# OpenVVC/OpenVVC

Hardware: AMD Instinct MI355X
Metric: decoded frames/sec, full rcn back-end decode step (H2D of the recorded picture + MC incl. BDOF/DMVR/affine-PROF/GPM/CIIP + LMCS + inverse transform + ordered intra pass + deblocking + SAO + ALF/CC-ALF + D2H of refined MVs + wait + per-picture digest + publication to the device DPB), 4K 10-bit RA rec (higher is better)
Workload: dtype u16 samples / int16 coefficients / int32 accumulate

## Files before the change

openvvc_amd/csrc/kernels_alf.hip:

```cpp
#include "ovvc_common.hip.h"

#ifndef OV_WPE_ALF
#define OV_WPE_ALF 0
#endif
#if OV_WPE_ALF > 0
#define OV_OCC_ALF __attribute__((amdgpu_waves_per_eu(OV_WPE_ALF)))
#else
#define OV_OCC_ALF
#endif

namespace {

#define TL 32
#define LH 3
#define LW (TL + 2 * LH)
#define LPAD 4
#define LWS 40
#define CH 2
#define CW (TL + 2 * CH)

struct AlfRect { int x0, y0, x1, y1; };
__device__ __forceinline__ AlfRect alf_clamp_rect(int border, int x0, int y0, int s, int w, int h)
{
    AlfRect r = { 0, 0, w - 1, h - 1 };
    if (border & OVHIP_BORDER_LEFT) r.x0 = x0;
    if (border & OVHIP_BORDER_UPPER) r.y0 = y0;
    if (border & OVHIP_BORDER_RIGHT) r.x1 = min(r.x1, x0 + s - 1);
    if (border & OVHIP_BORDER_BOTTOM) r.y1 = min(r.y1, y0 + s - 1);
    return r;
}

__device__ __forceinline__ int alf_clipd(int clip, int ref, int a, int b)
{
    return ov_clip3(a - ref, -clip, clip) + ov_clip3(b - ref, -clip, clip);
}

typedef short alf_s2 __attribute__((ext_vector_type(2)));
#define A6I(c) (((c) + 4) >> 1)
#define A6H(c) (((c) + 4) & 1)
#define A2I(c) ((c) >> 1)
#define A2H(c) ((c) & 1)
#define ALF_PK(da, ha, db, hb) __builtin_amdgcn_perm((db), (da), (uint32_t)((2 * (ha)) | ((2 * (ha) + 1) << 8) | ((4 + 2 * (hb)) << 16) | ((5 + 2 * (hb)) << 24)))
#define ALF_PK66(A, ca, B, cb) ALF_PK((A)[A6I(ca)], A6H(ca), (B)[A6I(cb)], A6H(cb))
#define ALF_PK22(A, ca, B, cb) ALF_PK((A)[A2I(ca)], A2H(ca), (B)[A2I(cb)], A2H(cb))
__device__ __forceinline__ uint32_t alf_dup(int v) { return __builtin_amdgcn_perm((uint32_t)v, (uint32_t)v, 0x01000100u); }
__device__ __forceinline__ int alf_tap(uint32_t pair, uint32_t cur2, uint32_t c2, uint32_t nc2, uint32_t f2, int sum)
{
    alf_s2 d = __builtin_bit_cast(alf_s2, pair) - __builtin_bit_cast(alf_s2, cur2);
    d = __builtin_elementwise_min(__builtin_elementwise_max(d, __builtin_bit_cast(alf_s2, nc2)), __builtin_bit_cast(alf_s2, c2));
    return __builtin_amdgcn_sdot2(d, __builtin_bit_cast(alf_s2, f2), sum, false);
}
__device__ __forceinline__ int alf_tap_lin(uint32_t pair, uint32_t f2, int sum)
{
    return __builtin_amdgcn_sdot2(__builtin_bit_cast(alf_s2, pair), __builtin_bit_cast(alf_s2, f2), sum, false);
}

__device__ __forceinline__ void filter_idx(uint32_t sum_h, uint32_t sum_v, uint32_t sum_d, uint32_t sum_b, bool is_vb,
                                           int &cls, int &tr)
{
    const uint32_t scale = is_vb ? 96u : 64u;
    const int act = min((int)(((sum_h + sum_v) * scale) >> (OV_BD + 4)), 15);
    int c = act == 0 ? 0 : act == 1 ? 1 : act <= 6 ? 2 : act <= 14 ? 3 : 4;
    uint32_t max_hv, min_hv, max_db, min_db, max_dir, min_dir;
    int dir_hv, dir_db, main_dir, sec_dir;
    if (sum_v > sum_h) { max_hv = sum_v; min_hv = sum_h; dir_hv = 1; } else { max_hv = sum_h; min_hv = sum_v; dir_hv = 3; }
    if (sum_d > sum_b) { max_db = sum_d; min_db = sum_b; dir_db = 0; } else { max_db = sum_b; min_db = sum_d; dir_db = 2; }
    if (max_db * min_hv > max_hv * min_db) { max_dir = max_db; min_dir = min_db; main_dir = dir_db; sec_dir = dir_hv; }
    else { max_dir = max_hv; min_dir = min_hv; main_dir = dir_hv; sec_dir = dir_db; }
    if (max_dir * 2 > 9 * min_dir) c += (((main_dir & 1) << 1) + 2) * 5;
    else if (max_dir > 2 * min_dir) c += (((main_dir & 1) << 1) + 1) * 5;
    cls = c;
    const int k = (main_dir << 1) + (sec_dir >> 1);
    tr = (0xDE84 >> (2 * k)) & 3;
}

__device__ __forceinline__ void alf_luma_tile(const ovhip_pic &dst, const ovhip_pic &src, const ovhip_alf_pic &alf, int nb_ctu_w,
                                              int tile0, uint16_t *s_t, uint8_t *s_cls, uint4 *s_sum, int row0, int row1)
{

    const int W = src.w, H = src.h;
    const int tid = threadIdx.x;
    const int ctu = 1 << alf.log2_ctu_s;
    const int ntx = (W + TL - 1) / TL, ntiles = ntx * ((H + TL - 1) / TL);
    for (int tile = tile0; tile < ntiles; tile = ntiles) {
    const int tx0 = (tile % ntx) * TL, ty0 = (tile / ntx) * TL;
    const ovhip_alf_ctu c = alf.ctus[(ty0 >> alf.log2_ctu_s) * nb_ctu_w + (tx0 >> alf.log2_ctu_s)];
    const bool on = c.flags & 4;

    const int b = tid >> 2, r = tid & 3;
    const int bx = (b & 7) * 4, by = (b >> 3) * 4;
    const int ox = tx0 + bx, oy = ty0 + by + r;

    if (!on) {
        if (oy < H && oy >= row0 && oy < row1) {
#pragma unroll
            for (int i = 0; i < 4; ++i) if (ox + i < W) dst.y[oy * dst.stride_y + ox + i] = src.y[oy * src.stride_y + ox + i];
        }
        continue;
    }

    const AlfRect rc = alf_clamp_rect(c.border, tx0 & ~(ctu - 1), ty0 & ~(ctu - 1), ctu, W, H);
    if (tx0 >= rc.x0 + LPAD && tx0 + TL + LPAD <= rc.x1 + 1 && ty0 >= rc.y0 + LH && ty0 + TL + LH <= rc.y1 + 1 && !(src.stride_y & 7)) {
        if (tid < LW * 5) {
            const int yy = tid / 5, q = tid - yy * 5;
            *reinterpret_cast<uint4 *>(s_t + yy * LWS + 8 * q) =
                *reinterpret_cast<const uint4 *>(src.y + (ty0 + yy - LH) * src.stride_y + tx0 - LPAD + 8 * q);
        }
    } else {
        for (int i = tid; i < LW * LWS; i += 256) {
            const int yy = i / LWS, xx = i - yy * LWS;
            const int sy = ov_clip3(ty0 + yy - LH, rc.y0, rc.y1), sx = ov_clip3(tx0 + xx - LPAD, rc.x0, rc.x1);
            s_t[i] = src.y[sy * src.stride_y + sx];
        }
    }
    __syncthreads();

    const int ctu_y0 = ty0 & ~(ctu - 1);
    const bool truncated = ctu_y0 + ctu > H;
    const int vbl = truncated ? H : ctu - 4;
    const int last_local = (ctu_y0 + (truncated ? H - ctu_y0 : ctu) - 1) & (ctu - 1);
    const bool req_vb = (last_local < vbl && last_local >= vbl - 4) || (last_local >= vbl && last_local <= vbl + 3);
    const int vb = ctu_y0 + vbl;

#define T(x, y) ((int)s_t[((y) + LH) * LWS + (x) + LPAD])
    {
        const int cb = tid >> 2, k = tid & 3;
        const int cbx = (cb & 7) * 4, cby = (cb >> 3) * 4;
        const int rr = cby - 2 + 2 * k;
        int above = rr - 1, below = rr + 2;
        if (ty0 + rr + 2 == vb) below = rr + 1;
        if (ty0 + rr == vb)     above = rr;
        uint32_t sv = 0, sh = 0, sd = 0, sb = 0;
        {
            uint32_t ra[6], r0[6], r1[6], rb[6];
            const uint16_t *base = s_t + LH * LWS + cbx;
            auto row3 = [&](int y, uint32_t d6[6]) {
                const uint2 *q2 = reinterpret_cast<const uint2 *>(base + y * LWS);
                const uint2 a = q2[0], b_ = q2[1], c_ = q2[2];
                d6[0] = a.x; d6[1] = a.y; d6[2] = b_.x; d6[3] = b_.y; d6[4] = c_.x; d6[5] = c_.y;
            };
            row3(above, ra); row3(rr, r0); row3(rr + 1, r1); row3(below, rb);
            typedef unsigned short alf_u2 __attribute__((ext_vector_type(2)));
#pragma unroll
            for (int q = 0; q < 4; ++q) {
                const int c0 = 2 * q - 2, c1 = c0 + 1;
                const alf_u2 ctr = __builtin_bit_cast(alf_u2, ALF_PK66(r0, c0, r1, c1));
                const uint32_t y2 = __builtin_bit_cast(uint32_t, ctr + ctr);
#define LAP(acc, A, ca, B, cb, C, cc_, D, cd)                                                                      \
                acc = __builtin_amdgcn_sad_u16(y2, __builtin_bit_cast(uint32_t, __builtin_bit_cast(alf_u2, ALF_PK66(A, ca, B, cb)) + \
                                                                               __builtin_bit_cast(alf_u2, ALF_PK66(C, cc_, D, cd))), acc)
                LAP(sv, ra, c0, r0, c1, r1, c0, rb, c1);
                LAP(sh, r0, c0 + 1, r1, c1 + 1, r0, c0 - 1, r1, c1 - 1);
                LAP(sd, ra, c0 - 1, r0, c1 - 1, r1, c0 + 1, rb, c1 + 1);
                LAP(sb, r1, c0 - 1, rb, c1 - 1, ra, c0 + 1, r0, c1 + 1);
#undef LAP
            }
        }
        const int py = ty0 + cby;
        bool use = true, is_vb = false;
        if (py == vb - 4) { is_vb = true; use = k < 3; }
        if (py == vb)     { is_vb = true; use = k > 0; }
        if (!use) sv = sh = sd = sb = 0;
        (void)is_vb;
        s_sum[tid] = make_uint4(sv, sh, sd, sb);
    }
    __syncthreads();
    if (tid < 64) {
        const uint4 p0 = s_sum[4 * tid], p1 = s_sum[4 * tid + 1], p2 = s_sum[4 * tid + 2], p3 = s_sum[4 * tid + 3];
        const int py = ty0 + (tid >> 3) * 4;
        int cls, tr;
        filter_idx(p0.y + p1.y + p2.y + p3.y, p0.x + p1.x + p2.x + p3.x, p0.z + p1.z + p2.z + p3.z, p0.w + p1.w + p2.w + p3.w,
                   py == vb - 4 || py == vb, cls, tr);
        s_cls[tid] = (uint8_t)(cls | (tr << 5));
    }
    __syncthreads();

    if (oy >= H || oy < row0 || oy >= row1) continue;
    const int ct = s_cls[b];
    const int cls = ct & 31, tr = ct >> 5;
    const int16_t *f = alf.luma_coeff + c.luma_set * OVHIP_ALF_LUMA_SET_SIZE + tr * 25 * 13 + cls * 13;
    const int16_t *cl = alf.luma_clip + c.luma_set * OVHIP_ALF_LUMA_SET_SIZE + tr * 25 * 13 + cls * 13;
    typedef uint32_t alf_u32a2 __attribute__((aligned(2)));
    uint32_t fw[6], cw6[6];
#pragma unroll
    for (int j = 0; j < 6; ++j) { fw[j] = *reinterpret_cast<const alf_u32a2 *>(f + 2 * j); cw6[j] = *reinterpret_cast<const alf_u32a2 *>(cl + 2 * j); }

    int d = 3;
    bool near = false;
    if (req_vb) {
        if (oy < vb && oy >= vb - 4) d = vb - 1 - oy;
        else if (oy >= vb && oy <= vb + 3) d = oy - vb;
        near = (oy == vb - 1) || (oy == vb);
    }
    const int o1 = min(d, 1), o2 = min(d, 2), o3 = min(d, 3);
    const int ly = by + r;
    uint32_t r0[6], p1[6], m1[6], p2[6], m2[6], p3[2], m3[2];
    {
        const uint16_t *base = s_t + LH * LWS + bx;
        auto row3 = [&](int y, uint32_t d6[6]) {
            const uint2 *q = reinterpret_cast<const uint2 *>(base + y * LWS);
            const uint2 a = q[0], b_ = q[1], c_ = q[2];
            d6[0] = a.x; d6[1] = a.y; d6[2] = b_.x; d6[3] = b_.y; d6[4] = c_.x; d6[5] = c_.y;
        };
        auto row1 = [&](int y, uint32_t d2[2]) {
            const uint2 a = reinterpret_cast<const uint2 *>(base + y * LWS)[1];
            d2[0] = a.x; d2[1] = a.y;
        };
        row3(ly, r0); row3(ly + o1, p1); row3(ly - o1, m1); row3(ly + o2, p2); row3(ly - o2, m2);
        row1(ly + o3, p3); row1(ly - o3, m3);
    }
#define S6(d6, c) ((((c) + 4) & 1) ? (int)((d6)[((c) + 4) >> 1] >> 16) : (int)((d6)[((c) + 4) >> 1] & 0xffff))
#define S2(d2, c) (((c) & 1) ? (int)((d2)[(c) >> 1] >> 16) : (int)((d2)[(c) >> 1] & 0xffff))
    alf_s2 cm2 = __builtin_bit_cast(alf_s2, cw6[0]);
    int fsum = 0;
#pragma unroll
    for (int j = 1; j < 6; ++j) cm2 = __builtin_elementwise_min(cm2, __builtin_bit_cast(alf_s2, cw6[j]));
#pragma unroll
    for (int j = 0; j < 6; ++j) fsum = __builtin_amdgcn_sdot2(__builtin_bit_cast(alf_s2, fw[j]), (alf_s2)(1), fsum, false);
    const int cmin = min((int)cm2.x, (int)cm2.y);
    const bool linear = __all(cmin > OV_PIX_MAX);
    uint32_t f2[12], c2[12], nc2[12];
#pragma unroll
    for (int j = 0; j < 6; ++j) {
        f2[2 * j] = __builtin_amdgcn_perm(fw[j], fw[j], 0x01000100u); f2[2 * j + 1] = __builtin_amdgcn_perm(fw[j], fw[j], 0x03020302u);
    }
    if (!linear) {
#pragma unroll
        for (int j = 0; j < 6; ++j) {
            c2[2 * j] = __builtin_amdgcn_perm(cw6[j], cw6[j], 0x01000100u); c2[2 * j + 1] = __builtin_amdgcn_perm(cw6[j], cw6[j], 0x03020302u);
        }
#pragma unroll
        for (int i = 0; i < 12; ++i) nc2[i] = __builtin_bit_cast(uint32_t, (alf_s2)(0) - __builtin_bit_cast(alf_s2, c2[i]));
    }
    int outv[4];
#pragma unroll
    for (int i = 0; i < 4; ++i) {
        const int cur = S6(r0, i);
        const uint32_t n[12] = {
            ALF_PK22(p3, i, m3, i),
            ALF_PK66(p2, i + 1, m2, i - 1), ALF_PK66(p2, i, m2, i), ALF_PK66(p2, i - 1, m2, i + 1),
            ALF_PK66(p1, i + 2, m1, i - 2), ALF_PK66(p1, i + 1, m1, i - 1), ALF_PK66(p1, i, m1, i),
            ALF_PK66(p1, i - 1, m1, i + 1), ALF_PK66(p1, i - 2, m1, i + 2),
            ALF_PK66(r0, i + 3, r0, i - 3), ALF_PK66(r0, i + 2, r0, i - 2), ALF_PK66(r0, i + 1, r0, i - 1) };
        int sum;
        if (linear) {
            sum = -2 * cur * fsum;
#pragma unroll
            for (int k = 0; k < 12; ++k) sum = alf_tap_lin(n[k], f2[k], sum);
        } else {
            const uint32_t cur2 = ALF_PK66(r0, i, r0, i);
            sum = 0;
#pragma unroll
            for (int k = 0; k < 12; ++k) sum = alf_tap(n[k], cur2, c2[k], nc2[k], f2[k], sum);
        }
        sum = near ? (sum + 512) >> 10 : (sum + 64) >> 7;
        outv[i] = ov_clip_bd(sum + cur);
    }
#undef S6
#undef S2
    {
        uint16_t *o = dst.y + oy * dst.stride_y + ox;
        if (ox + 3 < W && !(dst.stride_y & 3)) {
            uint2 v; v.x = (uint32_t)outv[0] | ((uint32_t)outv[1] << 16); v.y = (uint32_t)outv[2] | ((uint32_t)outv[3] << 16);
            *reinterpret_cast<uint2 *>(o) = v;
        } else {
#pragma unroll
            for (int i = 0; i < 4; ++i) if (ox + i < W) o[i] = (uint16_t)outv[i];
        }
    }
    }
#undef T
}

__device__ __forceinline__ void alf_chroma_tile(const ovhip_pic &dst, const ovhip_pic &src, const ovhip_alf_pic &alf, int nb_ctu_w,
                                                int tile0, int comp, uint16_t *s_t, int row0, int row1)
{
    const int W = src.w, H = src.h, Wc = W >> 1, Hc = H >> 1;
    const int tid = threadIdx.x;
    const int ctu = 1 << alf.log2_ctu_s, ctuc = ctu >> 1;
    const int ntx = (Wc + TL - 1) / TL, ntiles = ntx * ((Hc + TL - 1) / TL);
    for (int tile = tile0; tile < ntiles; tile = ntiles) {
    const int tx0 = (tile % ntx) * TL, ty0 = (tile / ntx) * TL;
    const ovhip_alf_ctu c = alf.ctus[((ty0 * 2) >> alf.log2_ctu_s) * nb_ctu_w + ((tx0 * 2) >> alf.log2_ctu_s)];
    const bool on = c.flags & (comp == 1 ? 2 : 1);
    const int cc_idx = comp == 1 ? c.cc_cb_idx : c.cc_cr_idx;
    const uint16_t *sp = comp == 1 ? src.cb : src.cr;
    uint16_t *dp = comp == 1 ? dst.cb : dst.cr;

    const AlfRect rcc = alf_clamp_rect(c.border, tx0 & ~(ctuc - 1), ty0 & ~(ctuc - 1), ctuc, Wc, Hc);
    if (on) {
        if (tx0 >= rcc.x0 + LPAD && tx0 + TL + LPAD <= rcc.x1 + 1 && ty0 >= rcc.y0 + CH && ty0 + TL + CH <= rcc.y1 + 1 && !(src.stride_c & 7)) {
            if (tid < CW * 5) {
                const int yy = tid / 5, q = tid - yy * 5;
                *reinterpret_cast<uint4 *>(s_t + yy * LWS + 8 * q) =
                    *reinterpret_cast<const uint4 *>(sp + (ty0 + yy - CH) * src.stride_c + tx0 - LPAD + 8 * q);
            }
        } else {
            for (int i = tid; i < CW * LWS; i += 256) {
                const int yy = i / LWS, xx = i - yy * LWS;
                const int sy = ov_clip3(ty0 + yy - CH, rcc.y0, rcc.y1), sx = ov_clip3(tx0 + xx - LPAD, rcc.x0, rcc.x1);
                s_t[i] = sp[sy * src.stride_c + sx];
            }
        }
        __syncthreads();
    }

    const int ctu_y0 = (ty0 * 2) & ~(ctu - 1);
    const bool truncated = ctu_y0 + ctu > H;
    int fc[6], cl[6];
    if (on) {
        const int alt = comp == 1 ? c.cb_alt : c.cr_alt;
#pragma unroll
        for (int i = 0; i < 6; ++i) { fc[i] = alf.chroma_coeff[alt * 7 + i]; cl[i] = alf.chroma_clip[alt * 7 + i]; }
    }
    int cf[7];
    if (cc_idx) {
#pragma unroll
        for (int i = 0; i < 7; ++i) cf[i] = alf.cc_coeff[((comp - 1) * 4 + (cc_idx - 1)) * 8 + i];
    }

    const int ly = tid >> 3, lx0 = (tid & 7) * 4;
    const int oy = ty0 + ly;
    if (oy >= Hc || oy < (row0 >> 1) || oy >= (row1 >> 1)) continue;
    int o1 = 1, o2 = 2;
    bool near = false;
    if (on) {
        const int vb = truncated ? H / 2 : (ctu - 4) / 2;
        const int yl = oy & (ctuc - 1);
        int d = 2;
        if (yl < vb && yl >= vb - 2) d = vb - 1 - yl;
        else if (yl >= vb && yl <= vb + 1) d = yl - vb;
        near = (yl == vb - 1) || (yl == vb);
        o1 = min(d, 1); o2 = min(d, 2);
    }
    int r1 = 1, r2 = -1, r3 = 2;
    if (cc_idx) {
        const int vbpos = truncated ? H / 2 : ctu - 4;
        const int pos = (oy << 1) & (ctu - 1);
        if (pos == vbpos - 2 || pos == vbpos + 1) r3 = r1;
        else if (pos == vbpos - 1 || pos == vbpos) r1 = r2 = r3 = 0;
    }
    const bool cc_inside = tx0 > rcc.x0 && ty0 > rcc.y0 && tx0 + TL <= rcc.x1 && ty0 + TL <= rcc.y1;
    const AlfRect rcl = { 2 * rcc.x0, 2 * rcc.y0, min(2 * rcc.x1 + 1, W - 1), min(2 * rcc.y1 + 1, H - 1) };
    uint32_t r0[6], p1[6], m1[6], p2[2], m2[2];
    int cmin = 0x7fff, fsum = 0;
    if (on) {
        const uint16_t *base = s_t + CH * LWS + lx0;
        auto row3 = [&](int y, uint32_t d6[6]) {
            const uint2 *q = reinterpret_cast<const uint2 *>(base + y * LWS);
            const uint2 a = q[0], b_ = q[1], c_ = q[2];
            d6[0] = a.x; d6[1] = a.y; d6[2] = b_.x; d6[3] = b_.y; d6[4] = c_.x; d6[5] = c_.y;
        };
        auto row1 = [&](int y, uint32_t d2[2]) {
            const uint2 a = reinterpret_cast<const uint2 *>(base + y * LWS)[1];
            d2[0] = a.x; d2[1] = a.y;
        };
        row3(ly, r0); row3(ly + o1, p1); row3(ly - o1, m1); row1(ly + o2, p2); row1(ly - o2, m2);
#pragma unroll
        for (int i = 0; i < 6; ++i) { cmin = min(cmin, cl[i]); fsum += fc[i]; }
    }
    const bool linear = on && cmin > OV_PIX_MAX;
    uint32_t f2[6], c2[6], nc2[6];
#pragma unroll
    for (int i = 0; i < 6; ++i) {
        f2[i] = alf_dup(fc[i]);
        c2[i] = alf_dup(cl[i]);
        nc2[i] = __builtin_bit_cast(uint32_t, (alf_s2)(0) - __builtin_bit_cast(alf_s2, c2[i]));
    }
#define S6(d6, c) ((((c) + 4) & 1) ? (int)((d6)[((c) + 4) >> 1] >> 16) : (int)((d6)[((c) + 4) >> 1] & 0xffff))
#define S2(d2, c) (((c) & 1) ? (int)((d2)[(c) >> 1] >> 16) : (int)((d2)[(c) >> 1] & 0xffff))
    int outv[4];
#pragma unroll
    for (int i = 0; i < 4; ++i) {
        const int ox = min(tx0 + lx0 + i, Wc - 1);
        int out;
        if (on) {
            const int cur = S6(r0, i);
            int sum;
            const uint32_t n[6] = { ALF_PK22(p2, i, m2, i),
                                    ALF_PK66(p1, i + 1, m1, i - 1), ALF_PK66(p1, i, m1, i), ALF_PK66(p1, i - 1, m1, i + 1),
                                    ALF_PK66(r0, i + 2, r0, i - 2), ALF_PK66(r0, i + 1, r0, i - 1) };
            if (linear) {
                sum = -2 * cur * fsum;
#pragma unroll
                for (int k = 0; k < 6; ++k) sum = alf_tap_lin(n[k], f2[k], sum);
            } else {
                const uint32_t cur2 = ALF_PK66(r0, i, r0, i);
                sum = 0;
#pragma unroll
                for (int k = 0; k < 6; ++k) sum = alf_tap(n[k], cur2, c2[k], nc2[k], f2[k], sum);
            }
            sum = near ? (sum + 512) >> 10 : (sum + 64) >> 7;
            out = ov_clip_bd(sum + cur);
        } else {
            out = sp[oy * src.stride_c + ox];
        }
        if (cc_idx) {
            const int Lx = ox << 1, Ly = oy << 1;
            int cy, sum = 0;
            if (cc_inside) {
                const uint16_t *lp = src.y + Ly * src.stride_y + Lx;
                cy = lp[0];
                sum += cf[0] * ((int)lp[r2 * src.stride_y] - cy);
                sum += cf[1] * ((int)lp[-1] - cy);
                sum += cf[2] * ((int)lp[1] - cy);
                sum += cf[3] * ((int)lp[r1 * src.stride_y - 1] - cy);
                sum += cf[4] * ((int)lp[r1 * src.stride_y] - cy);
                sum += cf[5] * ((int)lp[r1 * src.stride_y + 1] - cy);
                sum += cf[6] * ((int)lp[r3 * src.stride_y] - cy);
            } else {
#define LU(dx, dy) ((int)src.y[ov_clip3(Ly + (dy), rcl.y0, rcl.y1) * src.stride_y + ov_clip3(Lx + (dx), rcl.x0, rcl.x1)])
                cy = LU(0, 0);
                sum += cf[0] * (LU(0, r2) - cy);
                sum += cf[1] * (LU(-1, 0) - cy);
                sum += cf[2] * (LU(1, 0) - cy);
                sum += cf[3] * (LU(-1, r1) - cy);
                sum += cf[4] * (LU(0, r1) - cy);
                sum += cf[5] * (LU(1, r1) - cy);
                sum += cf[6] * (LU(0, r3) - cy);
#undef LU
            }
            sum = (sum + 64) >> 7;
            sum = ov_clip_bd(sum + (1 << OV_BD >> 1));
            out = ov_clip_bd(sum + out - (1 << OV_BD >> 1));
        }
        outv[i] = out;
    }
#undef S6
#undef S2
    uint16_t *o = dp + oy * dst.stride_c + tx0 + lx0;
    if (tx0 + lx0 + 3 < Wc && !(dst.stride_c & 3)) {
        uint2 v; v.x = (uint32_t)outv[0] | ((uint32_t)outv[1] << 16); v.y = (uint32_t)outv[2] | ((uint32_t)outv[3] << 16);
        *reinterpret_cast<uint2 *>(o) = v;
    } else {
#pragma unroll
        for (int i = 0; i < 4; ++i) if (tx0 + lx0 + i < Wc) o[i] = (uint16_t)outv[i];
    }
    }
}

__global__ __launch_bounds__(256) OV_OCC_ALF void k_alf(ovhip_pic dst, ovhip_pic src, ovhip_alf_pic alf, int nb_ctu_w, int nl, int nc, int t0_l, int t0_c, int row0, int row1)
{
    __shared__ __attribute__((aligned(16))) uint16_t s_t[(LW > CW ? LW : CW) * LWS];
    __shared__ uint8_t s_cls[64];
    __shared__ __attribute__((aligned(16))) uint4 s_sum[256];
    const int b = blockIdx.x;
    if (b < nl) alf_luma_tile(dst, src, alf, nb_ctu_w, t0_l + (int)ov_xcd_slot_at(b, 0, nl), s_t, s_cls, s_sum, row0, row1);
    else {
        const int comp = 1 + (b - nl) / nc;
        alf_chroma_tile(dst, src, alf, nb_ctu_w, t0_c + (int)ov_xcd_slot_at(b, nl + (comp - 1) * nc, nc), comp, s_t, row0, row1);
    }
}

}

extern "C" int ovhip_alf_launch_rows(ovhip_ctx *ctx, const ovhip_pic *dst, const ovhip_pic *src, const ovhip_alf_pic *alf, int32_t row0, int32_t row1)
{
    if (!ctx || !dst || !src || !alf) return OVHIP_EINVAL;
    OV_DEVICE(ctx);
    if (dst->w != src->w || dst->h != src->h || dst->y == src->y || alf->log2_ctu_s < 6 || alf->log2_ctu_s > 7 ||
        !alf->ctus || !alf->luma_coeff || !alf->luma_clip || !alf->chroma_coeff || !alf->chroma_clip || !alf->cc_coeff)
        return ov_fail(ctx, OVHIP_EINVAL, "ovhip_alf_launch: bad pictures / parameter tables", hipSuccess);
    if (row0 < 0 || row1 > src->h || row0 > row1 || (row0 & 7) || ((row1 & 7) && row1 != src->h))
        return ov_fail(ctx, OVHIP_EINVAL, "ovhip_alf_launch_rows: row window", hipSuccess);
    if (row0 == row1) return OVHIP_OK;
    const int nb_ctu_w = (src->w + (1 << alf->log2_ctu_s) - 1) >> alf->log2_ctu_s;
    const int ntx_l = (src->w + TL - 1) / TL, ntx_c = (src->w / 2 + TL - 1) / TL;
    const int ty0_l = row0 / TL, ty1_l = (row1 + TL - 1) / TL, ty0_c = (row0 / 2) / TL, ty1_c = (row1 / 2 + TL - 1) / TL;
    const int nl = ntx_l * (ty1_l - ty0_l), nc = ntx_c * (ty1_c - ty0_c);
    hipLaunchKernelGGL(k_alf, dim3(nl + 2 * nc), dim3(256), 0, ctx->stream, *dst, *src, *alf, nb_ctu_w, nl, nc, ty0_l * ntx_l, ty0_c * ntx_c, row0, row1);
    OV_LAUNCH_CHECK(ctx, "k_alf");
    return OVHIP_OK;
}

extern "C" int ovhip_alf_launch(ovhip_ctx *ctx, const ovhip_pic *dst, const ovhip_pic *src, const ovhip_alf_pic *alf)
{
    if (!src) return OVHIP_EINVAL;
    return ovhip_alf_launch_rows(ctx, dst, src, alf, 0, src->h);
}
```

Baseline: 3530.

## Restructure ALF kernel: shared Laplacian cells, per-block coeff sets, paired chroma with staged CC luma

Luma classification now computes Laplacian sums once per 4x2 cell over 162 threads and reuses them across overlapping 4x4 class windows. The 64 per-block coefficient/clip sets are pre-expanded once into LDS instead of being fetched and repacked from global memory by every thread. Chroma Cb and Cr now run in one block that shares a staged luma window in LDS for CC-ALF, replacing scattered global luma reads and halving the chroma block count. The cost is a larger unified LDS footprint, which may reduce occupancy, plus more complex indexing.

```diff
diff --git a/openvvc_amd/csrc/kernels_alf.hip b/openvvc_amd/csrc/kernels_alf.hip
--- a/openvvc_amd/csrc/kernels_alf.hip
+++ b/openvvc_amd/csrc/kernels_alf.hip
@@ -18,6 +18,21 @@
 #define LWS 40
 #define CH 2
 #define CW (TL + 2 * CH)
+#define ALF_NPAIR 18
+#define ALF_NCELL 9
+#define ALF_SETW 40
+#define CCPAD 8
+#define CCWS 80
+#define CCROWS 66
+#define ALF_S_T 0
+#define ALF_S_LAP (LW * LWS / 2)
+#define ALF_S_SET (ALF_S_LAP + 4 * ALF_NPAIR * ALF_NCELL)
+#define ALF_S_LUMA (ALF_S_SET + 64 * ALF_SETW)
+#define ALF_S_T2 (CW * LWS / 2)
+#define ALF_S_CC (2 * CW * LWS / 2)
+#define ALF_S_CHROMA (ALF_S_CC + CCROWS * CCWS / 2)
+#define ALF_S_DWORDS (ALF_S_LUMA > ALF_S_CHROMA ? ALF_S_LUMA : ALF_S_CHROMA)
+static_assert(!(ALF_S_LAP & 3) && !(ALF_S_SET & 3) && !(ALF_S_T2 & 3) && !(ALF_S_CC & 3), "k_alf LDS layout");
 
 struct AlfRect { int x0, y0, x1, y1; };
 __device__ __forceinline__ AlfRect alf_clamp_rect(int border, int x0, int y0, int s, int w, int h)
@@ -74,16 +89,23 @@
     tr = (0xDE84 >> (2 * k)) & 3;
 }
 
+__device__ __forceinline__ void alf_ld4(const uint4 *p, uint32_t *d) { const uint4 v = *p; d[0] = v.x; d[1] = v.y; d[2] = v.z; d[3] = v.w; }
+__device__ __forceinline__ uint32_t alf_pk2(int lo, int hi) { return ((uint32_t)lo & 0xffffu) | ((uint32_t)hi << 16); }
+
 __device__ __forceinline__ void alf_luma_tile(const ovhip_pic &dst, const ovhip_pic &src, const ovhip_alf_pic &alf, int nb_ctu_w,
-                                              int tile0, uint16_t *s_t, uint8_t *s_cls, uint4 *s_sum, int row0, int row1)
-{
+                                              int tile, uint32_t *s_mem, int row0, int row1)
+{
+    uint16_t *s_t = reinterpret_cast<uint16_t *>(s_mem + ALF_S_T);
+    uint4 *s_lap = reinterpret_cast<uint4 *>(s_mem + ALF_S_LAP);
+    uint32_t *s_set = s_mem + ALF_S_SET;
 
     const int W = src.w, H = src.h;
     const int tid = threadIdx.x;
     const int ctu = 1 << alf.log2_ctu_s;
-    const int ntx = (W + TL - 1) / TL, ntiles = ntx * ((H + TL - 1) / TL);
-    for (int tile = tile0; tile < ntiles; tile = ntiles) {
-    const int tx0 = (tile % ntx) * TL, ty0 = (tile / ntx) * TL;
+    const int ntx = (W + TL - 1) / TL;
+    if (tile >= ntx * ((H + TL - 1) / TL)) return;
+    const int tyi = tile / ntx;
+    const int tx0 = (tile - tyi * ntx) * TL, ty0 = tyi * TL;
     const ovhip_alf_ctu c = alf.ctus[(ty0 >> alf.log2_ctu_s) * nb_ctu_w + (tx0 >> alf.log2_ctu_s)];
     const bool on = c.flags & 4;
 
@@ -96,7 +118,7 @@
 #pragma unroll
             for (int i = 0; i < 4; ++i) if (ox + i < W) dst.y[oy * dst.stride_y + ox + i] = src.y[oy * src.stride_y + ox + i];
         }
-        continue;
+        return;
     }
 
     const AlfRect rc = alf_clamp_rect(c.border, tx0 & ~(ctu - 1), ty0 & ~(ctu - 1), ctu, W, H);
@@ -122,68 +144,86 @@
     const bool req_vb = (last_local < vbl && last_local >= vbl - 4) || (last_local >= vbl && last_local <= vbl + 3);
     const int vb = ctu_y0 + vbl;
 
-#define T(x, y) ((int)s_t[((y) + LH) * LWS + (x) + LPAD])
-    {
-        const int cb = tid >> 2, k = tid & 3;
-        const int cbx = (cb & 7) * 4, cby = (cb >> 3) * 4;
-        const int rr = cby - 2 + 2 * k;
+    if (tid < ALF_NPAIR * ALF_NCELL) {
+        const int p = tid / ALF_NCELL, j = tid - p * ALF_NCELL;
+        const int rr = 2 * p - 2;
         int above = rr - 1, below = rr + 2;
         if (ty0 + rr + 2 == vb) below = rr + 1;
         if (ty0 + rr == vb)     above = rr;
         uint32_t sv = 0, sh = 0, sd = 0, sb = 0;
-        {
-            uint32_t ra[6], r0[6], r1[6], rb[6];
-            const uint16_t *base = s_t + LH * LWS + cbx;
-            auto row3 = [&](int y, uint32_t d6[6]) {
-                const uint2 *q2 = reinterpret_cast<const uint2 *>(base + y * LWS);
-                const uint2 a = q2[0], b_ = q2[1], c_ = q2[2];
-                d6[0] = a.x; d6[1] = a.y; d6[2] = b_.x; d6[3] = b_.y; d6[4] = c_.x; d6[5] = c_.y;
-            };
-            row3(above, ra); row3(rr, r0); row3(rr + 1, r1); row3(below, rb);
-            typedef unsigned short alf_u2 __attribute__((ext_vector_type(2)));
-#pragma unroll
-            for (int q = 0; q < 4; ++q) {
-                const int c0 = 2 * q - 2, c1 = c0 + 1;
-                const alf_u2 ctr = __builtin_bit_cast(alf_u2, ALF_PK66(r0, c0, r1, c1));
-                const uint32_t y2 = __builtin_bit_cast(uint32_t, ctr + ctr);
+        uint32_t ra[4], r0[4], r1[4], rb[4];
+        const uint16_t *base = s_t + LH * LWS + 4 * j;
+        auto row2 = [&](int y, uint32_t d4[4]) {
+            const uint2 *q2 = reinterpret_cast<const uint2 *>(base + y * LWS);
+            const uint2 a = q2[0], b_ = q2[1];
+            d4[0] = a.x; d4[1] = a.y; d4[2] = b_.x; d4[3] = b_.y;
+        };
+        row2(above, ra); row2(rr, r0); row2(rr + 1, r1); row2(below, rb);
+        typedef unsigned short alf_u2 __attribute__((ext_vector_type(2)));
+#pragma unroll
+        for (int q = 0; q < 2; ++q) {
+            const int c0 = 2 * q - 2, c1 = c0 + 1;
+            const alf_u2 ctr = __builtin_bit_cast(alf_u2, ALF_PK66(r0, c0, r1, c1));
+            const uint32_t y2 = __builtin_bit_cast(uint32_t, ctr + ctr);
 #define LAP(acc, A, ca, B, cb, C, cc_, D, cd)                                                                      \
-                acc = __builtin_amdgcn_sad_u16(y2, __builtin_bit_cast(uint32_t, __builtin_bit_cast(alf_u2, ALF_PK66(A, ca, B, cb)) + \
-                                                                               __builtin_bit_cast(alf_u2, ALF_PK66(C, cc_, D, cd))), acc)
-                LAP(sv, ra, c0, r0, c1, r1, c0, rb, c1);
-                LAP(sh, r0, c0 + 1, r1, c1 + 1, r0, c0 - 1, r1, c1 - 1);
-                LAP(sd, ra, c0 - 1, r0, c1 - 1, r1, c0 + 1, rb, c1 + 1);
-                LAP(sb, r1, c0 - 1, rb, c1 - 1, ra, c0 + 1, r0, c1 + 1);
+            acc = __builtin_amdgcn_sad_u16(y2, __builtin_bit_cast(uint32_t, __builtin_bit_cast(alf_u2, ALF_PK66(A, ca, B, cb)) + \
+                                                                           __builtin_bit_cast(alf_u2, ALF_PK66(C, cc_, D, cd))), acc)
+            LAP(sv, ra, c0, r0, c1, r1, c0, rb, c1);
+            LAP(sh, r0, c0 + 1, r1, c1 + 1, r0, c0 - 1, r1, c1 - 1);
+            LAP(sd, ra, c0 - 1, r0, c1 - 1, r1, c0 + 1, rb, c1 + 1);
+            LAP(sb, r1, c0 - 1, rb, c1 - 1, ra, c0 + 1, r0, c1 + 1);
 #undef LAP
-            }
-        }
-        const int py = ty0 + cby;
-        bool use = true, is_vb = false;
-        if (py == vb - 4) { is_vb = true; use = k < 3; }
-        if (py == vb)     { is_vb = true; use = k > 0; }
-        if (!use) sv = sh = sd = sb = 0;
-        (void)is_vb;
-        s_sum[tid] = make_uint4(sv, sh, sd, sb);
+        }
+        s_lap[tid] = make_uint4(sv, sh, sd, sb);
     }
     __syncthreads();
     if (tid < 64) {
-        const uint4 p0 = s_sum[4 * tid], p1 = s_sum[4 * tid + 1], p2 = s_sum[4 * tid + 2], p3 = s_sum[4 * tid + 3];
-        const int py = ty0 + (tid >> 3) * 4;
+        const int bxi = tid & 7, byi = tid >> 3;
+        const int py = ty0 + byi * 4;
+        const bool at_above = py == vb - 4, at_below = py == vb;
+        uint32_t sv = 0, sh = 0, sd = 0, sb = 0;
+#pragma unroll
+        for (int k = 0; k < 4; ++k) {
+            const uint4 a = s_lap[(2 * byi + k) * ALF_NCELL + bxi], b_ = s_lap[(2 * byi + k) * ALF_NCELL + bxi + 1];
+            const bool use = !((k == 3 && at_above) || (k == 0 && at_below));
+            sv += use ? a.x + b_.x : 0u; sh += use ? a.y + b_.y : 0u; sd += use ? a.z + b_.z : 0u; sb += use ? a.w + b_.w : 0u;
+        }
         int cls, tr;
-        filter_idx(p0.y + p1.y + p2.y + p3.y, p0.x + p1.x + p2.x + p3.x, p0.z + p1.z + p2.z + p3.z, p0.w + p1.w + p2.w + p3.w,
-                   py == vb - 4 || py == vb, cls, tr);
-        s_cls[tid] = (uint8_t)(cls | (tr << 5));
+        filter_idx(sh, sv, sd, sb, at_above || at_below, cls, tr);
+        const int at = c.luma_set * OVHIP_ALF_LUMA_SET_SIZE + (tr * 25 + cls) * 13;
+        typedef uint32_t alf_u32a2 __attribute__((aligned(2)));
+        uint32_t w[ALF_SETW];
+        int fsum = 0;
+        alf_s2 cm2 = (alf_s2)(0x7fff);
+#pragma unroll
+        for (int j = 0; j < 6; ++j) {
+            const uint32_t fw = *reinterpret_cast<const alf_u32a2 *>(alf.luma_coeff + at + 2 * j), cw = *reinterpret_cast<const alf_u32a2 *>(alf.luma_clip + at + 2 * j);
+            fsum = __builtin_amdgcn_sdot2(__builtin_bit_cast(alf_s2, fw), (alf_s2)(1), fsum, false);
+            cm2 = __builtin_elementwise_min(cm2, __builtin_bit_cast(alf_s2, cw));
+            w[2 * j] = __builtin_amdgcn_perm(fw, fw, 0x01000100u); w[2 * j + 1] = __builtin_amdgcn_perm(fw, fw, 0x03020302u);
+            w[12 + 2 * j] = __builtin_amdgcn_perm(cw, cw, 0x01000100u); w[13 + 2 * j] = __builtin_amdgcn_perm(cw, cw, 0x03020302u);
+        }
+#pragma unroll
+        for (int i = 0; i < 12; ++i) w[24 + i] = __builtin_bit_cast(uint32_t, (alf_s2)(0) - __builtin_bit_cast(alf_s2, w[12 + i]));
+        const int cmin = min((int)cm2.x, (int)cm2.y);
+        w[36] = (uint32_t)fsum; w[37] = cmin > OV_PIX_MAX; w[38] = w[39] = 0;
+        uint4 *st = reinterpret_cast<uint4 *>(s_set + tid * ALF_SETW);
+#pragma unroll
+        for (int i = 0; i < ALF_SETW / 4; ++i) st[i] = make_uint4(w[4 * i], w[4 * i + 1], w[4 * i + 2], w[4 * i + 3]);
     }
     __syncthreads();
 
-    if (oy >= H || oy < row0 || oy >= row1) continue;
-    const int ct = s_cls[b];
-    const int cls = ct & 31, tr = ct >> 5;
-    const int16_t *f = alf.luma_coeff + c.luma_set * OVHIP_ALF_LUMA_SET_SIZE + tr * 25 * 13 + cls * 13;
-    const int16_t *cl = alf.luma_clip + c.luma_set * OVHIP_ALF_LUMA_SET_SIZE + tr * 25 * 13 + cls * 13;
-    typedef uint32_t alf_u32a2 __attribute__((aligned(2)));
-    uint32_t fw[6], cw6[6];
-#pragma unroll
-    for (int j = 0; j < 6; ++j) { fw[j] = *reinterpret_cast<const alf_u32a2 *>(f + 2 * j); cw6[j] = *reinterpret_cast<const alf_u32a2 *>(cl + 2 * j); }
+    if (oy >= H || oy < row0 || oy >= row1) return;
+    const uint4 *st = reinterpret_cast<const uint4 *>(s_set + b * ALF_SETW);
+    uint32_t f2[12], c2[12], nc2[12];
+    alf_ld4(st, f2); alf_ld4(st + 1, f2 + 4); alf_ld4(st + 2, f2 + 8);
+    const uint4 tail = st[9];
+    const int fsum = (int)tail.x;
+    const bool linear = __all(tail.y != 0);
+    if (!linear) {
+        alf_ld4(st + 3, c2); alf_ld4(st + 4, c2 + 4); alf_ld4(st + 5, c2 + 8);
+        alf_ld4(st + 6, nc2); alf_ld4(st + 7, nc2 + 4); alf_ld4(st + 8, nc2 + 8);
+    }
 
     int d = 3;
     bool near = false;
@@ -210,28 +250,6 @@
         row1(ly + o3, p3); row1(ly - o3, m3);
     }
 #define S6(d6, c) ((((c) + 4) & 1) ? (int)((d6)[((c) + 4) >> 1] >> 16) : (int)((d6)[((c) + 4) >> 1] & 0xffff))
-#define S2(d2, c) (((c) & 1) ? (int)((d2)[(c) >> 1] >> 16) : (int)((d2)[(c) >> 1] & 0xffff))
-    alf_s2 cm2 = __builtin_bit_cast(alf_s2, cw6[0]);
-    int fsum = 0;
-#pragma unroll
-    for (int j = 1; j < 6; ++j) cm2 = __builtin_elementwise_min(cm2, __builtin_bit_cast(alf_s2, cw6[j]));
-#pragma unroll
-    for (int j = 0; j < 6; ++j) fsum = __builtin_amdgcn_sdot2(__builtin_bit_cast(alf_s2, fw[j]), (alf_s2)(1), fsum, false);
-    const int cmin = min((int)cm2.x, (int)cm2.y);
-    const bool linear = __all(cmin > OV_PIX_MAX);
-    uint32_t f2[12], c2[12], nc2[12];
-#pragma unroll
-    for (int j = 0; j < 6; ++j) {
-        f2[2 * j] = __builtin_amdgcn_perm(fw[j], fw[j], 0x01000100u); f2[2 * j + 1] = __builtin_amdgcn_perm(fw[j], fw[j], 0x03020302u);
-    }
-    if (!linear) {
-#pragma unroll
-        for (int j = 0; j < 6; ++j) {
-            c2[2 * j] = __builtin_amdgcn_perm(cw6[j], cw6[j], 0x01000100u); c2[2 * j + 1] = __builtin_amdgcn_perm(cw6[j], cw6[j], 0x03020302u);
-        }
-#pragma unroll
-        for (int i = 0; i < 12; ++i) nc2[i] = __builtin_bit_cast(uint32_t, (alf_s2)(0) - __builtin_bit_cast(alf_s2, c2[i]));
-    }
     int outv[4];
 #pragma unroll
     for (int i = 0; i < 4; ++i) {
@@ -257,75 +275,84 @@
         outv[i] = ov_clip_bd(sum + cur);
     }
 #undef S6
-#undef S2
-    {
-        uint16_t *o = dst.y + oy * dst.stride_y + ox;
-        if (ox + 3 < W && !(dst.stride_y & 3)) {
-            uint2 v; v.x = (uint32_t)outv[0] | ((uint32_t)outv[1] << 16); v.y = (uint32_t)outv[2] | ((uint32_t)outv[3] << 16);
-            *reinterpret_cast<uint2 *>(o) = v;
-        } else {
-#pragma unroll
-            for (int i = 0; i < 4; ++i) if (ox + i < W) o[i] = (uint16_t)outv[i];
-        }
-    }
-    }
-#undef T
-}
-
-__device__ __forceinline__ void alf_chroma_tile(const ovhip_pic &dst, const ovhip_pic &src, const ovhip_alf_pic &alf, int nb_ctu_w,
-                                                int tile0, int comp, uint16_t *s_t, int row0, int row1)
-{
-    const int W = src.w, H = src.h, Wc = W >> 1, Hc = H >> 1;
+    uint16_t *o = dst.y + oy * dst.stride_y + ox;
+    if (ox + 3 < W && !(dst.stride_y & 3)) {
+        uint2 v; v.x = (uint32_t)outv[0] | ((uint32_t)outv[1] << 16); v.y = (uint32_t)outv[2] | ((uint32_t)outv[3] << 16);
+        *reinterpret_cast<uint2 *>(o) = v;
+    } else {
+#pragma unroll
+        for (int i = 0; i < 4; ++i) if (ox + i < W) o[i] = (uint16_t)outv[i];
+    }
+}
+
+struct AlfChromaTile {
+    int tx0, ty0;
+    ovhip_alf_ctu c;
+    AlfRect rcc;
+    bool truncated;
+};
+
+__device__ __forceinline__ void alf_chroma_stage(const ovhip_pic &src, const uint16_t *sp, const AlfChromaTile &t, uint16_t *s_t)
+{
+    const int tid = threadIdx.x;
+    if (t.tx0 >= t.rcc.x0 + LPAD && t.tx0 + TL + LPAD <= t.rcc.x1 + 1 && t.ty0 >= t.rcc.y0 + CH && t.ty0 + TL + CH <= t.rcc.y1 + 1 && !(src.stride_c & 7)) {
+        if (tid < CW * 5) {
+            const int yy = tid / 5, q = tid - yy * 5;
+            *reinterpret_cast<uint4 *>(s_t + yy * LWS + 8 * q) =
+                *reinterpret_cast<const uint4 *>(sp + (t.ty0 + yy - CH) * src.stride_c + t.tx0 - LPAD + 8 * q);
+        }
+    } else {
+        for (int i = tid; i < CW * LWS; i += 256) {
+            const int yy = i / LWS, xx = i - yy * LWS;
+            const int sy = ov_clip3(t.ty0 + yy - CH, t.rcc.y0, t.rcc.y1), sx = ov_clip3(t.tx0 + xx - LPAD, t.rcc.x0, t.rcc.x1);
+            s_t[i] = sp[sy * src.stride_c + sx];
+        }
+    }
+}
+
+__device__ __forceinline__ void alf_chroma_plane(const ovhip_pic &dst, const ovhip_pic &src, const ovhip_alf_pic &alf, const AlfChromaTile &t,
+                                                 int comp, const uint16_t *s_t, const uint16_t *s_cc, int row0, int row1)
+{
+    const int H = src.h, Wc = src.w >> 1, Hc = H >> 1;
     const int tid = threadIdx.x;
     const int ctu = 1 << alf.log2_ctu_s, ctuc = ctu >> 1;
-    const int ntx = (Wc + TL - 1) / TL, ntiles = ntx * ((Hc + TL - 1) / TL);
-    for (int tile = tile0; tile < ntiles; tile = ntiles) {
-    const int tx0 = (tile % ntx) * TL, ty0 = (tile / ntx) * TL;
-    const ovhip_alf_ctu c = alf.ctus[((ty0 * 2) >> alf.log2_ctu_s) * nb_ctu_w + ((tx0 * 2) >> alf.log2_ctu_s)];
-    const bool on = c.flags & (comp == 1 ? 2 : 1);
-    const int cc_idx = comp == 1 ? c.cc_cb_idx : c.cc_cr_idx;
+    const int tx0 = t.tx0, ty0 = t.ty0;
+    const bool on = t.c.flags & (comp == 1 ? 2 : 1);
+    const int cc_idx = comp == 1 ? t.c.cc_cb_idx : t.c.cc_cr_idx;
     const uint16_t *sp = comp == 1 ? src.cb : src.cr;
     uint16_t *dp = comp == 1 ? dst.cb : dst.cr;
 
-    const AlfRect rcc = alf_clamp_rect(c.border, tx0 & ~(ctuc - 1), ty0 & ~(ctuc - 1), ctuc, Wc, Hc);
-    if (on) {
-        if (tx0 >= rcc.x0 + LPAD && tx0 + TL + LPAD <= rcc.x1 + 1 && ty0 >= rcc.y0 + CH && ty0 + TL + CH <= rcc.y1 + 1 && !(src.stride_c & 7)) {
-            if (tid < CW * 5) {
-                const int yy = tid / 5, q = tid - yy * 5;
-                *reinterpret_cast<uint4 *>(s_t + yy * LWS + 8 * q) =
-                    *reinterpret_cast<const uint4 *>(sp + (ty0 + yy - CH) * src.stride_c + tx0 - LPAD + 8 * q);
-            }
-        } else {
-            for (int i = tid; i < CW * LWS; i += 256) {
-                const int yy = i / LWS, xx = i - yy * LWS;
-                const int sy = ov_clip3(ty0 + yy - CH, rcc.y0, rcc.y1), sx = ov_clip3(tx0 + xx - LPAD, rcc.x0, rcc.x1);
-                s_t[i] = sp[sy * src.stride_c + sx];
-            }
-        }
-        __syncthreads();
-    }
-
-    const int ctu_y0 = (ty0 * 2) & ~(ctu - 1);
-    const bool truncated = ctu_y0 + ctu > H;
-    int fc[6], cl[6];
-    if (on) {
-        const int alt = comp == 1 ? c.cb_alt : c.cr_alt;
-#pragma unroll
-        for (int i = 0; i < 6; ++i) { fc[i] = alf.chroma_coeff[alt * 7 + i]; cl[i] = alf.chroma_clip[alt * 7 + i]; }
-    }
-    int cf[7];
-    if (cc_idx) {
-#pragma unroll
-        for (int i = 0; i < 7; ++i) cf[i] = alf.cc_coeff[((comp - 1) * 4 + (cc_idx - 1)) * 8 + i];
-    }
-
     const int ly = tid >> 3, lx0 = (tid & 7) * 4;
     const int oy = ty0 + ly;
-    if (oy >= Hc || oy < (row0 >> 1) || oy >= (row1 >> 1)) continue;
+    if (oy >= Hc || oy < (row0 >> 1) || oy >= (row1 >> 1)) return;
+
+    uint32_t f2[6], c2[6], nc2[6];
+    int cmin = 0x7fff, fsum = 0;
+    if (on) {
+        const int alt = comp == 1 ? t.c.cb_alt : t.c.cr_alt;
+#pragma unroll
+        for (int i = 0; i < 6; ++i) {
+            const int fc = alf.chroma_coeff[alt * 7 + i], cl = alf.chroma_clip[alt * 7 + i];
+            cmin = min(cmin, cl); fsum += fc;
+            f2[i] = alf_pk2(fc, fc); c2[i] = alf_pk2(cl, cl); nc2[i] = alf_pk2(-cl, -cl);
+        }
+    }
+    const bool linear = on && cmin > OV_PIX_MAX;
+    uint32_t k_cr = 0, k_r1 = 0, k_l = 0, k_v = 0;
+    if (cc_idx) {
+        int cf[7], cs = 0;
+#pragma unroll
+        for (int i = 0; i < 7; ++i) { cf[i] = alf.cc_coeff[((comp - 1) * 4 + (cc_idx - 1)) * 8 + i]; cs += cf[i]; }
+        k_cr = alf_pk2(-cs, cf[2]);
+        k_r1 = alf_pk2(cf[4], cf[5]);
+        k_l = alf_pk2(cf[1], cf[3]);
+        k_v = alf_pk2(cf[0], cf[6]);
+    }
+
     int o1 = 1, o2 = 2;
     bool near = false;
     if (on) {
-        const int vb = truncated ? H / 2 : (ctu - 4) / 2;
+        const int vb = t.truncated ? H / 2 : (ctu - 4) / 2;
         const int yl = oy & (ctuc - 1);
         int d = 2;
         if (yl < vb && yl >= vb - 2) d = vb - 1 - yl;
@@ -333,17 +360,7 @@
         near = (yl == vb - 1) || (yl == vb);
         o1 = min(d, 1); o2 = min(d, 2);
     }
-    int r1 = 1, r2 = -1, r3 = 2;
-    if (cc_idx) {
-        const int vbpos = truncated ? H / 2 : ctu - 4;
-        const int pos = (oy << 1) & (ctu - 1);
-        if (pos == vbpos - 2 || pos == vbpos + 1) r3 = r1;
-        else if (pos == vbpos - 1 || pos == vbpos) r1 = r2 = r3 = 0;
-    }
-    const bool cc_inside = tx0 > rcc.x0 && ty0 > rcc.y0 && tx0 + TL <= rcc.x1 && ty0 + TL <= rcc.y1;
-    const AlfRect rcl = { 2 * rcc.x0, 2 * rcc.y0, min(2 * rcc.x1 + 1, W - 1), min(2 * rcc.y1 + 1, H - 1) };
     uint32_t r0[6], p1[6], m1[6], p2[2], m2[2];
-    int cmin = 0x7fff, fsum = 0;
     if (on) {
         const uint16_t *base = s_t + CH * LWS + lx0;
         auto row3 = [&](int y, uint32_t d6[6]) {
@@ -356,23 +373,24 @@
             d2[0] = a.x; d2[1] = a.y;
         };
         row3(ly, r0); row3(ly + o1, p1); row3(ly - o1, m1); row1(ly + o2, p2); row1(ly - o2, m2);
-#pragma unroll
-        for (int i = 0; i < 6; ++i) { cmin = min(cmin, cl[i]); fsum += fc[i]; }
-    }
-    const bool linear = on && cmin > OV_PIX_MAX;
-    uint32_t f2[6], c2[6], nc2[6];
-#pragma unroll
-    for (int i = 0; i < 6; ++i) {
-        f2[i] = alf_dup(fc[i]);
-        c2[i] = alf_dup(cl[i]);
-        nc2[i] = __builtin_bit_cast(uint32_t, (alf_s2)(0) - __builtin_bit_cast(alf_s2, c2[i]));
+    }
+    uint32_t l0[5], l1[5], l2[4], l3[4];
+    if (cc_idx) {
+        int r1 = 1, r2 = -1, r3 = 2;
+        const int vbpos = t.truncated ? H / 2 : ctu - 4;
+        const int pos = (oy << 1) & (ctu - 1);
+        if (pos == vbpos - 2 || pos == vbpos + 1) r3 = r1;
+        else if (pos == vbpos - 1 || pos == vbpos) r1 = r2 = r3 = 0;
+        const uint16_t *lb = s_cc + (2 * ly + 1) * CCWS + CCPAD + 2 * lx0;
+        l0[0] = *reinterpret_cast<const uint32_t *>(lb - 2);             alf_ld4(reinterpret_cast<const uint4 *>(lb), l0 + 1);
+        l1[0] = *reinterpret_cast<const uint32_t *>(lb + r1 * CCWS - 2); alf_ld4(reinterpret_cast<const uint4 *>(lb + r1 * CCWS), l1 + 1);
+        alf_ld4(reinterpret_cast<const uint4 *>(lb + r2 * CCWS), l2);
+        alf_ld4(reinterpret_cast<const uint4 *>(lb + r3 * CCWS), l3);
     }
 #define S6(d6, c) ((((c) + 4) & 1) ? (int)((d6)[((c) + 4) >> 1] >> 16) : (int)((d6)[((c) + 4) >> 1] & 0xffff))
-#define S2(d2, c) (((c) & 1) ? (int)((d2)[(c) >> 1] >> 16) : (int)((d2)[(c) >> 1] & 0xffff))
     int outv[4];
 #pragma unroll
     for (int i = 0; i < 4; ++i) {
-        const int ox = min(tx0 + lx0 + i, Wc - 1);
         int out;
         if (on) {
             const int cur = S6(r0, i);
@@ -393,33 +411,13 @@
             sum = near ? (sum + 512) >> 10 : (sum + 64) >> 7;
             out = ov_clip_bd(sum + cur);
         } else {
-            out = sp[oy * src.stride_c + ox];
+            out = sp[oy * src.stride_c + min(tx0 + lx0 + i, Wc - 1)];
         }
         if (cc_idx) {
-            const int Lx = ox << 1, Ly = oy << 1;
-            int cy, sum = 0;
-            if (cc_inside) {
-                const uint16_t *lp = src.y + Ly * src.stride_y + Lx;
-                cy = lp[0];
-                sum += cf[0] * ((int)lp[r2 * src.stride_y] - cy);
-                sum += cf[1] * ((int)lp[-1] - cy);
-                sum += cf[2] * ((int)lp[1] - cy);
-                sum += cf[3] * ((int)lp[r1 * src.stride_y - 1] - cy);
-                sum += cf[4] * ((int)lp[r1 * src.stride_y] - cy);
-                sum += cf[5] * ((int)lp[r1 * src.stride_y + 1] - cy);
-                sum += cf[6] * ((int)lp[r3 * src.stride_y] - cy);
-            } else {
-#define LU(dx, dy) ((int)src.y[ov_clip3(Ly + (dy), rcl.y0, rcl.y1) * src.stride_y + ov_clip3(Lx + (dx), rcl.x0, rcl.x1)])
-                cy = LU(0, 0);
-                sum += cf[0] * (LU(0, r2) - cy);
-                sum += cf[1] * (LU(-1, 0) - cy);
-                sum += cf[2] * (LU(1, 0) - cy);
-                sum += cf[3] * (LU(-1, r1) - cy);
-                sum += cf[4] * (LU(0, r1) - cy);
-                sum += cf[5] * (LU(1, r1) - cy);
-                sum += cf[6] * (LU(0, r3) - cy);
-#undef LU
-            }
+            int sum = alf_tap_lin(l0[1 + i], k_cr, 0);
+            sum = alf_tap_lin(l1[1 + i], k_r1, sum);
+            sum = alf_tap_lin(ALF_PK(l0[i], 1, l1[i], 1), k_l, sum);
+            sum = alf_tap_lin(ALF_PK(l2[i], 0, l3[i], 0), k_v, sum);
             sum = (sum + 64) >> 7;
             sum = ov_clip_bd(sum + (1 << OV_BD >> 1));
             out = ov_clip_bd(sum + out - (1 << OV_BD >> 1));
@@ -427,7 +425,6 @@
         outv[i] = out;
     }
 #undef S6
-#undef S2
     uint16_t *o = dp + oy * dst.stride_c + tx0 + lx0;
     if (tx0 + lx0 + 3 < Wc && !(dst.stride_c & 3)) {
         uint2 v; v.x = (uint32_t)outv[0] | ((uint32_t)outv[1] << 16); v.y = (uint32_t)outv[2] | ((uint32_t)outv[3] << 16);
@@ -436,20 +433,55 @@
 #pragma unroll
         for (int i = 0; i < 4; ++i) if (tx0 + lx0 + i < Wc) o[i] = (uint16_t)outv[i];
     }
-    }
+}
+
+__device__ __forceinline__ void alf_chroma_pair(const ovhip_pic &dst, const ovhip_pic &src, const ovhip_alf_pic &alf, int nb_ctu_w,
+                                                int tile, uint32_t *s_mem, int row0, int row1)
+{
+    uint16_t *s_cb = reinterpret_cast<uint16_t *>(s_mem + ALF_S_T), *s_cr = reinterpret_cast<uint16_t *>(s_mem + ALF_S_T2);
+    uint16_t *s_cc = reinterpret_cast<uint16_t *>(s_mem + ALF_S_CC);
+    const int W = src.w, H = src.h, Wc = W >> 1, Hc = H >> 1;
+    const int tid = threadIdx.x;
+    const int ctu = 1 << alf.log2_ctu_s, ctuc = ctu >> 1;
+    const int ntx = (Wc + TL - 1) / TL;
+    if (tile >= ntx * ((Hc + TL - 1) / TL)) return;
+    const int tyi = tile / ntx;
+    AlfChromaTile t;
+    t.tx0 = (tile - tyi * ntx) * TL; t.ty0 = tyi * TL;
+    t.c = alf.ctus[((t.ty0 * 2) >> alf.log2_ctu_s) * nb_ctu_w + ((t.tx0 * 2) >> alf.log2_ctu_s)];
+    t.rcc = alf_clamp_rect(t.c.border, t.tx0 & ~(ctuc - 1), t.ty0 & ~(ctuc - 1), ctuc, Wc, Hc);
+    t.truncated = ((t.ty0 * 2) & ~(ctu - 1)) + ctu > H;
+
+    if (t.c.flags & 2) alf_chroma_stage(src, src.cb, t, s_cb);
+    if (t.c.flags & 1) alf_chroma_stage(src, src.cr, t, s_cr);
+    if (t.c.cc_cb_idx | t.c.cc_cr_idx) {
+        const AlfRect rcl = { 2 * t.rcc.x0, 2 * t.rcc.y0, min(2 * t.rcc.x1 + 1, W - 1), min(2 * t.rcc.y1 + 1, H - 1) };
+        const int lx0 = 2 * t.tx0 - CCPAD, ly0 = 2 * t.ty0 - 1;
+        if (lx0 >= rcl.x0 && lx0 + CCWS <= rcl.x1 + 1 && ly0 >= rcl.y0 && ly0 + CCROWS <= rcl.y1 + 1 && !(src.stride_y & 7)) {
+            for (int i = tid; i < CCROWS * (CCWS / 8); i += 256) {
+                const int yy = i / (CCWS / 8), q = i - yy * (CCWS / 8);
+                *reinterpret_cast<uint4 *>(s_cc + yy * CCWS + 8 * q) =
+                    *reinterpret_cast<const uint4 *>(src.y + (ly0 + yy) * src.stride_y + lx0 + 8 * q);
+            }
+        } else {
+            for (int i = tid; i < CCROWS * CCWS; i += 256) {
+                const int yy = i / CCWS, xx = i - yy * CCWS;
+                const int sy = ov_clip3(ly0 + yy, rcl.y0, rcl.y1), sx = ov_clip3(lx0 + xx, rcl.x0, rcl.x1);
+                s_cc[i] = src.y[sy * src.stride_y + sx];
+            }
+        }
+    }
+    __syncthreads();
+    alf_chroma_plane(dst, src, alf, t, 1, s_cb, s_cc, row0, row1);
+    alf_chroma_plane(dst, src, alf, t, 2, s_cr, s_cc, row0, row1);
 }
 
 __global__ __launch_bounds__(256) OV_OCC_ALF void k_alf(ovhip_pic dst, ovhip_pic src, ovhip_alf_pic alf, int nb_ctu_w, int nl, int nc, int t0_l, int t0_c, int row0, int row1)
 {
-    __shared__ __attribute__((aligned(16))) uint16_t s_t[(LW > CW ? LW : CW) * LWS];
-    __shared__ uint8_t s_cls[64];
-    __shared__ __attribute__((aligned(16))) uint4 s_sum[256];
+    __shared__ __attribute__((aligned(16))) uint32_t s_mem[ALF_S_DWORDS];
     const int b = blockIdx.x;
-    if (b < nl) alf_luma_tile(dst, src, alf, nb_ctu_w, t0_l + (int)ov_xcd_slot_at(b, 0, nl), s_t, s_cls, s_sum, row0, row1);
-    else {
-        const int comp = 1 + (b - nl) / nc;
-        alf_chroma_tile(dst, src, alf, nb_ctu_w, t0_c + (int)ov_xcd_slot_at(b, nl + (comp - 1) * nc, nc), comp, s_t, row0, row1);
-    }
+    if (b < nl) alf_luma_tile(dst, src, alf, nb_ctu_w, t0_l + (int)ov_xcd_slot_at(b, 0, nl), s_mem, row0, row1);
+    else alf_chroma_pair(dst, src, alf, nb_ctu_w, t0_c + (int)ov_xcd_slot_at(b, nl, nc), s_mem, row0, row1);
 }
 
 }
@@ -468,7 +500,7 @@
     const int ntx_l = (src->w + TL - 1) / TL, ntx_c = (src->w / 2 + TL - 1) / TL;
     const int ty0_l = row0 / TL, ty1_l = (row1 + TL - 1) / TL, ty0_c = (row0 / 2) / TL, ty1_c = (row1 / 2 + TL - 1) / TL;
     const int nl = ntx_l * (ty1_l - ty0_l), nc = ntx_c * (ty1_c - ty0_c);
-    hipLaunchKernelGGL(k_alf, dim3(nl + 2 * nc), dim3(256), 0, ctx->stream, *dst, *src, *alf, nb_ctu_w, nl, nc, ty0_l * ntx_l, ty0_c * ntx_c, row0, row1);
+    hipLaunchKernelGGL(k_alf, dim3(nl + nc), dim3(256), 0, ctx->stream, *dst, *src, *alf, nb_ctu_w, nl, nc, ty0_l * ntx_l, ty0_c * ntx_c, row0, row1);
     OV_LAUNCH_CHECK(ctx, "k_alf");
     return OVHIP_OK;
 }
```

New measurement: 3572, median of 6. Within noise of the previous version (+1.2%).
